# gabrielcheda/optimized-rag

Measured on AMD Instinct MI355X. Metric: queries/sec + p50 retrieve+rerank latency, 1536-d top-k=20, higher is better.
Workload: dtype f16 MFMA + block-scaled bf8 MFMA corrections (fp32 acc) in the cross-encoder; f16 MFMA pass + f64 rescore in the dense leg; f64 BM25 / RRF; 1 GPU; 1000000 docs x 1536-d + BM25 postings (2M-term Zipf vocabulary) + 224-token passage store; batch=256 queries: dense top-100 + BM25 top-100 + RRF -> top-100 -> ms-marco-MiniLM-L-6 cross-encoder (L=256, 25,600 pairs, seeded weights) -> top-20 (BASELINE.json configs[3]); corpus_rows=1000000, rows_per_gpu=1000000, batch_queries=256, pool=100, k=20, parallelism=one rag_retrieve_rerank_dev call per batch, exchange=single process

## Files before the change

optimized-rag_amd/csrc/api.hip:

```cpp
#include "common.h"

#include <cctype>
#include <cmath>
#include <cstdlib>
#include <cstring>

static thread_local std::string g_null_err = "null handle";

static const struct { const char* name; int rag_options::*field; } g_options[] = {
    {"force_level", &rag_options::force_level},         {"stage_growth", &rag_options::stage_growth},
    {"no_smallq", &rag_options::no_smallq},             {"no_second_pass", &rag_options::no_second_pass},
    {"dense_linear_order", &rag_options::dense_linear_order}, {"dense_persist", &rag_options::dense_persist},
    {"bm25_first_ranges", &rag_options::bm25_first_ranges}, {"bm25_no_staging", &rag_options::bm25_no_staging},
    {"bm25_packed", &rag_options::bm25_packed},         {"bm25_plan_slots", &rag_options::bm25_plan_slots},       {"bm25_ws_mb", &rag_options::bm25_ws_mb},
    {"bm25_tail_fold", &rag_options::bm25_tail_fold},     {"bm25_keep_tf", &rag_options::bm25_keep_tf},
    {"sparse_tail_fold", &rag_options::sparse_tail_fold}, {"tokvec_compact_rows", &rag_options::tokvec_compact_rows},
    {"bm25_linear_grid", &rag_options::bm25_linear_grid},            {"bm25_sort_merge", &rag_options::bm25_sort_merge},
    {"no_fork", &rag_options::no_fork},                 {"fork_max_q", &rag_options::fork_max_q},
    {"ce_chunk_tokens", &rag_options::ce_chunk_tokens}, {"ce_mx", &rag_options::ce_mx},
    {"ce_attn_stream", &rag_options::ce_attn_stream},
};
static void options_from_env(rag_options* o) {
    for (const auto& e : g_options) {
        std::string env = "RAG_";
        for (const char* c = e.name; *c; ++c) env += (char)toupper(*c);
        if (const char* v = getenv(env.c_str())) o->*(e.field) = atoi(v);
    }
}
#define DEV_ENTRY(h)                                                                           \
    do {                                                                                      \
        HIP_TRY(h, hipSetDevice((h)->device));                                                \
        (h)->dev_pending = true;                                                              \
    } while (0)
#define HOST_ENTRY(h)                                                                          \
    do {                                                                                      \
        HIP_TRY(h, hipSetDevice((h)->device));                                                \
        if (int rc_ = host_after_dev(h)) return rc_;                                          \
    } while (0)

struct entry_tenants { int tenant; query_tenants qt; };
static int entry_tenants_of(rag_ctx* h, int tenant, const int32_t* tenants_host, int Q, hipStream_t st, entry_tenants* out) {
    *out = {tenant, {nullptr, nullptr}};
    if (tenants_host == nullptr) return RAG_OK;
    const int32_t t0 = std::max(tenants_host[0], -1);
    bool uniform = true;
    for (int q = 1; q < Q && uniform; ++q) uniform = std::max(tenants_host[q], -1) == t0;
    out->tenant = t0;
    return uniform ? RAG_OK : stage_query_tenants(h, tenants_host, Q, st, &out->qt);
}

template <class T>
static int pairwise_cosine_host_t(rag_handle_t h, const T* a, int m, const T* b, int n, int dim, double* out) {
    if (!h) return RAG_ERR_ARG;
    LOCK(h);
    ARG_CHECK(h, m >= 0 && n >= 0 && dim > 0, "bad sizes");
    if (m == 0 || n == 0) return RAG_OK;
    ARG_CHECK(h, a && b && out, "null pointer");
    HOST_ENTRY(h);
    const bool same = (a == b && m == n);
    hipStream_t st = h->stream;
    int rc = stage_reserve(h, stage_size((size_t)m * dim, sizeof(T)) + stage_size(same ? 0 : (size_t)n * dim, sizeof(T)) + stage_size((size_t)m * n, 8));
    if (rc) return rc;
    char* p = h->stage;
    T* ad = stage_take<T>(p, (size_t)m * dim);
    T* bd = same ? ad : stage_take<T>(p, (size_t)n * dim);
    double* od = stage_take<double>(p, (size_t)m * n);
    HIP_TRY(h, hipMemcpyAsync(ad, a, (size_t)m * dim * sizeof(T), hipMemcpyHostToDevice, st));
    if (!same) HIP_TRY(h, hipMemcpyAsync(bd, b, (size_t)n * dim * sizeof(T), hipMemcpyHostToDevice, st));
    if constexpr (sizeof(T) == 8) rc = pairwise_cosine_f64(h, ad, m, bd, n, dim, od, st);
    else rc = pairwise_cosine(h, ad, m, bd, n, dim, od, st);
    if (rc) return rc;
    HIP_TRY(h, hipMemcpyAsync(out, od, (size_t)m * n * sizeof(double), hipMemcpyDeviceToHost, st));
    HIP_TRY(h, hipStreamSynchronize(st));
// ... 1411 lines not shown
```

optimized-rag_amd/csrc/ce_mx.h:

```cpp
#pragma once
#include "common.h"

typedef int mx_v8i __attribute__((ext_vector_type(8)));
typedef int mx_v4i __attribute__((ext_vector_type(4)));

#define MX_TM 384
#define MX_TN 128
#define MX_A_PLANE (MX_TM * 16)
#define MX_B_PLANE (MX_TN * 16)
#define MX_A_STAGE (6 * MX_A_PLANE)
#define MX_B_STAGE (6 * MX_B_PLANE)
#define MX_STAGE (MX_A_STAGE + MX_B_STAGE)
#define MX_STAGES 3
#define MX_LDS (MX_STAGES * MX_STAGE)
#ifndef MX_HI8_TRUNCATE
#define MX_LO_SCALE 2048.0f
#else
#define MX_LO_SCALE (2048.0f * 1.0928961748633879f)
#endif
#define MX_SCALE_A 116
#define MX_SCALE_B 127

__host__ __device__ __forceinline__ int mx_hi_off(int rows, int r, int e) {
    const int j = e >> 4, h = (e >> 2) & 1, i = ((e >> 3) & 1) * 4 + (e & 3);
// ... 29 lines not shown

__device__ __forceinline__ mx_v4i mx_hi8(half8 f0, half8 f1) {
    const mx_v4i a = __builtin_bit_cast(mx_v4i, f0), b = __builtin_bit_cast(mx_v4i, f1);
    return (mx_v4i){mx_top4(a[0], a[1]), mx_top4(b[0], b[1]), mx_top4(a[2], a[3]), mx_top4(b[2], b[3])};
}
__device__ __forceinline__ mx_v8i mx_cat(mx_v4i lo, mx_v4i hi) { return (mx_v8i){lo[0], lo[1], lo[2], lo[3], hi[0], hi[1], hi[2], hi[3]}; }

template <bool SWAP>
__device__ __forceinline__ void mx_block(f32x16& acc, half8 wh0, half8 wh1, mx_v8i w8, half8 xh0, half8 xh1, mx_v8i x8) {
    if (!SWAP) {
        acc = __builtin_amdgcn_mfma_f32_32x32x16_f16(wh0, xh0, acc, 0, 0, 0);
        acc = __builtin_amdgcn_mfma_f32_32x32x16_f16(wh1, xh1, acc, 0, 0, 0);
        acc = __builtin_amdgcn_mfma_scale_f32_32x32x64_f8f6f4(w8, x8, acc, 1, 1, 0, MX_SCALE_A, 0, MX_SCALE_B);
    } else {
        acc = __builtin_amdgcn_mfma_f32_32x32x16_f16(xh0, wh0, acc, 0, 0, 0);
        acc = __builtin_amdgcn_mfma_f32_32x32x16_f16(xh1, wh1, acc, 0, 0, 0);
        acc = __builtin_amdgcn_mfma_scale_f32_32x32x64_f8f6f4(x8, w8, acc, 1, 1, 0, MX_SCALE_B, 0, MX_SCALE_A);
    }
}

__device__ __forceinline__ void mx_bdma(__amdgpu_buffer_rsrc_t rs, unsigned voff, unsigned soff, char* lds_uniform) {
    __builtin_amdgcn_raw_ptr_buffer_load_lds(rs, (__attribute__((address_space(3))) void*)lds_uniform, 16, voff, soff, 0, 0);
}

#define MX_BAR __builtin_amdgcn_s_barrier(); __builtin_amdgcn_sched_barrier(0);
#ifndef MX_ISSUE_W
#define MX_ISSUE_W(...) mx_bdma(__VA_ARGS__)
#endif
#ifndef MX_ISSUE_X
#define MX_ISSUE_X(...) mx_bdma(__VA_ARGS__)
#endif
#ifndef MX_BLOCK
#define MX_BLOCK(SWAP, ...) mx_block<SWAP>(__VA_ARGS__)
#endif
#ifndef MX_W_HI8
#define MX_W_HI8(h0, h1, lo) mx_hi8(h0, h1)
#endif
#ifndef MX_READ_A_IF
#define MX_READ_A_IF(b) true
#endif
#ifndef MX_STEP_WAIT
#define MX_STEP_WAIT "s_waitcnt vmcnt(6)"
#endif

struct mx_tile_iter {
    int n_ft, n_tt, xcd, n_slots, work;
    __device__ __forceinline__ int tt() const { return (work / n_ft) * 8 + xcd; }
    __device__ __forceinline__ int ft() const { return work % n_ft; }
    __device__ __forceinline__ bool valid() const { return tt() < n_tt; }
};

struct mx_stream {
    __amdgpu_buffer_rsrc_t w_rs, x_cur, x_nxt;
    unsigned w_cur, w_nxt, voff;
    int wid, ring, nk, a_off, b_off;
    bool has_next;
    char* smem;
};

#define MX_PIECE(S, k, st_, ws_, xrs_, ks_)                                                                               \
    {                                                                                                                     \
        const int p_ = (S).wid + 8 * (k);                                                                                 \
        if (p_ < 36) { MX_ISSUE_W((S).w_rs, (S).voff, (ws_) + (ks_) * MX_A_STAGE + p_ * 1024, (st_) + p_ * 1024); }         \
        else { MX_ISSUE_X(xrs_, (S).voff, (ks_) * MX_B_STAGE + (p_ - 36) * 1024, (st_) + p_ * 1024); }                     \
    }

template <bool SWAP>
__device__ __forceinline__ void mx_ksteps(f32x16 (&acc)[6], const mx_stream& S, bool first) {
    const int nk = S.nk;
    for (int t = 0; t < nk; ++t) {
        if (first || t > 0) asm volatile(MX_STEP_WAIT ::: "memory");
        MX_BAR
        const char* st = S.smem + ((S.ring + t) % MX_STAGES) * MX_STAGE;
        const int u2 = t + 2;
        const bool nx_ = u2 >= nk && S.has_next;
        const unsigned ks_ = (unsigned)(u2 < nk ? u2 : (S.has_next ? u2 - nk : nk - 1));
        char* const dst = S.smem + ((S.ring + u2) % MX_STAGES) * MX_STAGE;
        const unsigned wsrc = nx_ ? S.w_nxt : S.w_cur;
        const __amdgpu_buffer_rsrc_t xsrc = nx_ ? S.x_nxt : S.x_cur;
        const half8 xh0 = *reinterpret_cast<const half8*>(st + S.b_off);
        const half8 xh1 = *reinterpret_cast<const half8*>(st + S.b_off + 2 * MX_B_PLANE);
        const mx_v4i xl = *reinterpret_cast<const mx_v4i*>(st + S.b_off + 4 * MX_B_PLANE);
        half8 wh0[2], wh1[2];
        mx_v4i wl[2];
#define MX_READ_A(b, s)                                                                                               \
        wh0[s] = *reinterpret_cast<const half8*>(st + S.a_off + (b) * 512);                                            \
        wh1[s] = *reinterpret_cast<const half8*>(st + S.a_off + (b) * 512 + 2 * MX_A_PLANE);                           \
        wl[s] = *reinterpret_cast<const mx_v4i*>(st + S.a_off + (b) * 512 + 4 * MX_A_PLANE);
        MX_READ_A(0, 0)
        MX_READ_A(1, 1)
        const mx_v8i x8 = SWAP ? mx_cat(xl, mx_hi8(xh0, xh1)) : mx_cat(mx_hi8(xh0, xh1), xl);
#pragma unroll
        for (int b = 0; b < 6; ++b) {
            const mx_v4i w8h = MX_W_HI8(wh0[b & 1], wh1[b & 1], wl[b & 1]);
            const mx_v8i w8 = SWAP ? mx_cat(w8h, wl[b & 1]) : mx_cat(wl[b & 1], w8h);
            __builtin_amdgcn_sched_barrier(0);
            __builtin_amdgcn_s_setprio(1);
            MX_BLOCK(SWAP, acc[b], wh0[b & 1], wh1[b & 1], w8, xh0, xh1, x8);
            __builtin_amdgcn_s_setprio(0);
            __builtin_amdgcn_sched_barrier(0);
            if (b + 2 < 6 && MX_READ_A_IF(b + 2)) { MX_READ_A(b + 2, b & 1) }
            MX_PIECE(S, b, dst, wsrc, xsrc, ks_)
        }
#undef MX_READ_A
    }
}

template <class EPI>
__device__ __forceinline__ void mx_gemm_loop(const char* __restrict__ W, const char* __restrict__ X, int nk, int n_ft,
                                             int n_tt, char* smem, EPI& epi) {
    const int tid = threadIdx.x, lane = tid & 63;
    const int wid = __builtin_amdgcn_readfirstlane(tid >> 6);
    const int wm = wid >> 2, wn = wid & 3;
    mx_tile_iter it{n_ft, n_tt, (int)(blockIdx.x & 7), (int)(gridDim.x >> 3), (int)(blockIdx.x >> 3)};
    if (!it.valid()) return;
    const unsigned a_tile_b = (unsigned)nk * MX_A_STAGE, b_tile_b = (unsigned)nk * MX_B_STAGE;
    mx_stream S;
    S.voff = (unsigned)lane * 16u;
    S.wid = wid;
    S.nk = nk;
    S.smem = smem;
    S.ring = 0;
    S.w_rs = __builtin_amdgcn_make_buffer_rsrc(const_cast<char*>(W), 0, (int)((size_t)n_ft * a_tile_b), 0x00020000);
    S.x_cur = __builtin_amdgcn_make_buffer_rsrc(const_cast<char*>(X + (size_t)it.tt() * b_tile_b), 0, (int)b_tile_b, 0x00020000);
    S.x_nxt = S.x_cur;
    S.w_cur = (unsigned)it.ft() * a_tile_b;
    S.w_nxt = S.w_cur;
    S.has_next = false;
    S.a_off = (lane >> 5) * MX_A_PLANE + (wm * 192 + (lane & 31)) * 16;
    S.b_off = MX_A_STAGE + (lane >> 5) * MX_B_PLANE + (wn * 32 + (lane & 31)) * 16;
#pragma unroll
    for (int u = 0; u < 2; ++u) {
        char* st_ = smem + u * MX_STAGE;
#pragma unroll
        for (int k = 0; k < 6; ++k) MX_PIECE(S, k, st_, S.w_cur, S.x_cur, (unsigned)u)
    }
    epi.prepare(smem + MX_LDS);
    asm volatile("s_waitcnt lgkmcnt(0)" ::: "memory");
    MX_BAR
    for (bool first = true;; first = false) {
        {
            mx_tile_iter nx = it;
            nx.work += it.n_slots;
            S.has_next = nx.valid();
            if (S.has_next) {
                S.w_nxt = (unsigned)nx.ft() * a_tile_b;
                S.x_nxt = __builtin_amdgcn_make_buffer_rsrc(const_cast<char*>(X + (size_t)nx.tt() * b_tile_b), 0, (int)b_tile_b, 0x00020000);
            }
        }
        const bool swap = epi.swap_for(it.ft());
        f32x16 acc[6];
#pragma unroll
        for (int b = 0; b < 6; ++b)
#pragma unroll
            for (int r = 0; r < 16; ++r) acc[b][r] = 0.f;
        if (swap) mx_ksteps<true>(acc, S, first);
        else mx_ksteps<false>(acc, S, first);
        asm volatile("s_waitcnt vmcnt(0)" ::: "memory");
        MX_BAR
        epi(acc, it.tt(), it.ft(), swap, smem + MX_LDS);
        if (!S.has_next) break;
        it.work += it.n_slots;
        S.w_cur = S.w_nxt;
        S.x_cur = S.x_nxt;
        S.ring = (S.ring + nk) % MX_STAGES;
    }
    asm volatile("s_waitcnt vmcnt(0)" ::: "memory");
}

#define MX_PARAM_OFF 2048
__device__ __forceinline__ void mx_stage_params(float* dst, const float* __restrict__ src, int n) {
    for (int i = threadIdx.x; i < n; i += blockDim.x) dst[i] = src[i];
}
typedef unsigned mx_u2 __attribute__((ext_vector_type(2)));
typedef unsigned mx_u4 __attribute__((ext_vector_type(4)));

__device__ __forceinline__ size_t mx_img_base(int64_t m, int k, int nk) { return ((size_t)(m >> 7) * nk + (k >> 5)) * MX_B_STAGE; }

typedef short mx_s2 __attribute__((ext_vector_type(2)));
typedef float mx_f2 __attribute__((ext_vector_type(2)));
#ifndef MX_HI8_TRUNCATE
__device__ __forceinline__ void mx_split4(float v0, float v1, float v2, float v3, mx_u2& hi, unsigned& lo) {
    const half4 h = {(half_t)v0, (half_t)v1, (half_t)v2, (half_t)v3};
    hi = __builtin_bit_cast(mx_u2, h);
    float neg1;
    asm volatile("s_mov_b32 %0, 0xbf800000" : "=s"(neg1));
    const float l0 = __builtin_fmaf((float)h[0], neg1, v0), l1 = __builtin_fmaf((float)h[1], neg1, v1);
    const float l2 = __builtin_fmaf((float)h[2], neg1, v2), l3 = __builtin_fmaf((float)h[3], neg1, v3);
// ... 307 lines not shown
                const half8 rj = (q >> 1) ? r1 : r0;
                const half4 rh = (q & 1) ? (half4){rj[4], rj[5], rj[6], rj[7]} : (half4){rj[0], rj[1], rj[2], rj[3]};
                const unsigned rl = rl4[(q & 1) * 2 + (q >> 1)];
                float res[4];
                mx_join4(rh, rl, res);
                acc[b][q * 4] += bv.x + res[0];
                acc[b][q * 4 + 1] += bv.y + res[1];
                acc[b][q * 4 + 2] += bv.z + res[2];
                acc[b][q * 4 + 3] += bv.w + res[3];
                sm += (acc[b][q * 4] + acc[b][q * 4 + 1]) + (acc[b][q * 4 + 2] + acc[b][q * 4 + 3]);
            }
        }
        const float m_l = sm * (1.0f / 96.0f);
#pragma unroll
        for (int b = 0; b < 6; ++b)
#pragma unroll
            for (int r = 0; r < 16; ++r) { const float d = acc[b][r] - m_l; sq = fmaf(d, d, sq); }
        const float m_o = __shfl_xor(m_l, 32), sq_o = __shfl_xor(sq, 32);
        const float m_w = 0.5f * (m_l + m_o);
        const float sq_w = (sq + sq_o) + (m_l - m_o) * (m_l - m_o) * 48.0f;
        if (hh == 0) { st_sum[li] = m_w; st_sq[li] = sq_w; }
        asm volatile("s_waitcnt lgkmcnt(0)" ::: "memory");
        MX_BAR
        const float m_p = pr_sum[li], sq_p = pr_sq[li];
        const float mu = 0.5f * (m_w + m_p);
        const float var = ((sq_w + sq_p) + (m_w - m_p) * (m_w - m_p) * 96.0f) * (1.0f / H);
        const float rs = 1.0f / sqrtf(var + eps);
#pragma unroll
        for (int b = 0; b < 6; ++b) {
            const int f0 = wm * 192 + b * 32;
            float v[16];
#pragma unroll
            for (int q = 0; q < 4; ++q) {
                const float4 gv = *reinterpret_cast<const float4*>(gamma + f0 + 8 * q + 4 * hh);
                const float4 be = *reinterpret_cast<const float4*>(beta + f0 + 8 * q + 4 * hh);
                v[q * 4] = fmaf(acc[b][q * 4] - mu, rs * gv.x, be.x);
                v[q * 4 + 1] = fmaf(acc[b][q * 4 + 1] - mu, rs * gv.y, be.y);
                v[q * 4 + 2] = fmaf(acc[b][q * 4 + 2] - mu, rs * gv.z, be.z);
                v[q * 4 + 3] = fmaf(acc[b][q * 4 + 3] - mu, rs * gv.w, be.w);
            }
            mx_store_block(tile + (size_t)(f0 >> 5) * MX_B_STAGE, trow, hh, v);
        }
    }
};

template <class EPI>
__global__ __launch_bounds__(512) void mx_gemm_kernel(const char* __restrict__ W, const char* __restrict__ X, int nk, int n_ft,
                                                       const int32_t* __restrict__ m_packed, EPI epi) {
    extern __shared__ __attribute__((aligned(16))) char smem[];
    const int n_tt = (m_packed[0] + MX_TN - 1) / MX_TN;
    mx_gemm_loop(W, X, nk, n_ft, n_tt, smem, epi);
}
#define MX_KERNEL_LDS (MX_LDS + MX_PARAM_OFF + 6144)
```

optimized-rag_amd/csrc/common.h:

```cpp
#pragma once
#include <hip/hip_runtime.h>
#include <stdint.h>
#include <mutex>
#include <string>
#include <unordered_map>
#include <vector>

#include "../../include/rag_hip.h"

typedef _Float16 half_t;
typedef _Float16 half8 __attribute__((ext_vector_type(8)));
typedef _Float16 half4 __attribute__((ext_vector_type(4)));
typedef float f32x4 __attribute__((ext_vector_type(4)));
typedef float f32x16 __attribute__((ext_vector_type(16)));

#define RAG_CAND_CAP 4096
#define RAG_STAGE0_ROWS 2048
#define RAG_STAGE_GROWTH 8
#define RAG_TILE 256
#define RAG_BK 64
#define RAG_MAX_K 256
#define RAG_SCALE_LOG2 7

#define RAG_PROF_STAGES 3
struct rag_ce_model;
struct rag_bm25_index;
struct rag_ctx;

template <class T>
struct dev_buf {
    dev_buf() = default;
    dev_buf(dev_buf&& o) noexcept : p_(o.p_), n_(o.n_) { o.p_ = nullptr; o.n_ = 0; }
    dev_buf& operator=(dev_buf&& o) noexcept {
        if (this != &o) { reset(); p_ = o.p_; n_ = o.n_; o.p_ = nullptr; o.n_ = 0; }
        return *this;
    }
    ~dev_buf() { reset(); }
    void reset() {
        if (p_) (void)hipFree(p_);
        p_ = nullptr;
        n_ = 0;
    }
    int alloc(rag_ctx* h, size_t n);
    int reserve(rag_ctx* h, size_t n) { return n <= n_ ? RAG_OK : alloc(h, n); }
    operator T*() const { return p_; }
    T* get() const { return p_; }
    size_t size() const { return n_; }

private:
    T* p_ = nullptr;
    size_t n_ = 0;
};

struct rag_options {
    int force_level = 0;
    int stage_growth = 0;
    int no_smallq = 0;
    int no_second_pass = 0;
    int dense_persist = 0;
    int dense_linear_order = 0;
    int bm25_first_ranges = 0;
    int bm25_no_staging = 0;
    int bm25_linear_grid = 0;
    int bm25_sort_merge = 0;
    int bm25_plan_slots = 0;
    int bm25_ws_mb = 0;
    int bm25_packed = 0;
    int bm25_keep_tf = 0;
    int bm25_tail_fold = 0;
    int sparse_tail_fold = 0;
    int tokvec_compact_rows = 0;
    int no_fork = 0;
    int fork_max_q = 0;
    int ce_chunk_tokens = 0;
    int ce_mx = 0;
    int ce_attn_stream = 0;
};

struct dense_ws {
    dev_buf<half_t> q16;
    dev_buf<uint64_t> cand;
    dev_buf<unsigned> cnt;
    dev_buf<float> tau;
    dev_buf<float> bound;
    dev_buf<int> n_sorted;
    int alloc(rag_ctx* h, size_t rows, hipStream_t st);
};

struct rag_index_mem {
    dev_buf<float> emb32;
    dev_buf<half_t> emb16;
    dev_buf<int64_t> ids;
    dev_buf<int32_t> tenants;
    dev_buf<int> bad_rows;
    dev_buf<char> scan_scores;
    dev_buf<int32_t> tenant_tiles;
    dev_buf<int32_t> vis;
};
struct rag_device_mem : rag_index_mem {
    dev_buf<double> side_scores;
    dev_buf<double> temporal;
    dev_buf<char> lin_ws;
    dense_ws ws;
    dev_buf<float> q32;
    dev_buf<double> exact;
    dev_buf<int> flag;
    dev_buf<int> scan_list;
    dev_buf<int> stats;
    dense_ws ws_ovf;
    dev_buf<int> ovf_list;
    dev_buf<char> stage;
    dev_buf<uint16_t> tok;
    dev_buf<uint8_t> tok_hi;
    dev_buf<int32_t> tok_len;
    dev_buf<int> tok_bad;
    dev_buf<char> pipe_ws;
    dev_buf<int32_t> qten;
    dev_buf<int32_t> union_tiles;
    dev_buf<half_t> tv;
    dev_buf<uint8_t> tv8;
    dev_buf<int64_t> tv_off;
    dev_buf<int> tv_bad;
    dev_buf<char> tv_ws;
};

struct rag_ctx : rag_device_mem {
    int device = 0;
    int n_cu = 0;
    int dim = 0;
    int dim_pad = 0;
    hipStream_t stream = nullptr;
    hipStream_t side_stream = nullptr;
    hipEvent_t ev_fork = nullptr, ev_join = nullptr;
    std::string err;
    rag_options opt;
    bool profiling = false;
    void* comm = nullptr;
    int comm_rank = 0, comm_world = 1;

    int64_t n_rows = 0, id_base = 0;
    bool index_loaded = false;
    int64_t n_reserved = 0;
    double temporal_absmax = 0.0;
    struct { bool on = false; int Q = 0; int64_t n_rows = 0; int tenant = -1; std::vector<int32_t> tenants; } lin_begun;
    std::unordered_map<int32_t, std::pair<int64_t, int>> tenant_span;
    std::unordered_map<int32_t, std::vector<int32_t>> tenant_lists;
    int64_t tenant_rows = 0;
    int64_t n_deleted = 0;
    bool bm25_stale = false;
    bool bm25_compacted = false;

    bool dev_pending = false;
    int ws_q = 0;
    int q16_dirty = 0;
    std::mutex mu;

    struct prof_spans { std::vector<std::pair<hipEvent_t, hipEvent_t>> ev; int used = 0; };
    prof_spans prof[RAG_PROF_STAGES];
    rag_dense_stats last_stats = {};
    bool last_stats_valid = false;
    int last_q = 0, last_k = 0, last_stages = 0, last_shortlist = 0;
    double last_eps = 0;

    rag_bm25_index* bm25 = nullptr;
    rag_bm25_index* sparse = nullptr;
    bool sparse_stale = false;
    bool sparse_compacted = false;
    int64_t tok_rows = 0;
    int tok_L = 0;
    int64_t tv_docs = 0, tv_rows = 0;
    int64_t tv_docs_cap = 0, tv_rows_cap = 0;
    int tv_dim = 0;
    int tv_form = 0;
    bool tv_stale = false;
    int pair_format = RAG_PAIR_BERT;
    int attr_dense_emit_lds[2][2][2] = {}, attr_dense_persist_lds[2] = {}, attr_dense_select_lds = 0, attr_bm25_lds = 0;
    int attr_ce_gemm_lds = 0, attr_ce_mx_lds = 0;
    int attr_ce_attn_lds[2][3] = {};
    int attr_ce_attn64_lds = 0;
    int attr_ce_attn64s_lds = 0;
    int attr_m3_gemm_lds = 0;
    int attr_m3_compact_lds = 0;
    rag_ce_model* ce = nullptr;
    rag_ce_model* emb = nullptr;
};

#define HIP_TRY(h, expr)                                                                      \
    do {                                                                                      \
        hipError_t _e = (expr);                                                               \
        if (_e != hipSuccess) {                                                               \
            (h)->err = std::string(#expr) + ": " + hipGetErrorString(_e);                     \
            return RAG_ERR_HIP;                                                               \
        }                                                                                     \
    } while (0)

template <class T>
int dev_buf<T>::alloc(rag_ctx* h, size_t n) {
    reset();
    HIP_TRY(h, hipMalloc(&p_, n * sizeof(T)));
    n_ = n;
    return RAG_OK;
}

inline int dense_ws::alloc(rag_ctx* h, size_t rows, hipStream_t st) {
    int rc;
    if ((rc = q16.alloc(h, rows * h->dim_pad))) return rc;
    if ((rc = cand.alloc(h, rows * RAG_CAND_CAP))) return rc;
    if ((rc = cnt.alloc(h, rows))) return rc;
    if ((rc = tau.alloc(h, 2 * rows))) return rc;
    if ((rc = bound.alloc(h, rows))) return rc;
    if ((rc = n_sorted.alloc(h, rows))) return rc;
    HIP_TRY(h, hipMemsetAsync(q16, 0, rows * h->dim_pad * sizeof(half_t), st));
    return RAG_OK;
}

#define LOCK(h) std::lock_guard<std::mutex> lock_((h)->mu)

enum { PLANE_EMB32, PLANE_EMB16, PLANE_IDS, PLANE_TENANTS, PLANE_TEMPORAL, PLANE_VIS, PLANE_TOK, PLANE_TOK_HI, PLANE_TOK_LEN };
template <class F>
static int for_each_row_plane(const rag_ctx* h, F&& f) {
    int rc;
    if ((rc = f(PLANE_EMB32, &rag_device_mem::emb32, (int64_t)h->dim))) return rc;
    if ((rc = f(PLANE_EMB16, &rag_device_mem::emb16, (int64_t)h->dim_pad))) return rc;
    if ((rc = f(PLANE_IDS, &rag_device_mem::ids, (int64_t)1))) return rc;
    if ((rc = f(PLANE_TENANTS, &rag_device_mem::tenants, (int64_t)1))) return rc;
    if ((rc = f(PLANE_TEMPORAL, &rag_device_mem::temporal, (int64_t)1))) return rc;
    if ((rc = f(PLANE_VIS, &rag_device_mem::vis, (int64_t)1))) return rc;
    if ((rc = f(PLANE_TOK, &rag_device_mem::tok, (int64_t)h->tok_L))) return rc;
    if ((rc = f(PLANE_TOK_HI, &rag_device_mem::tok_hi, (int64_t)h->tok_L))) return rc;
    return f(PLANE_TOK_LEN, &rag_device_mem::tok_len, (int64_t)1);
// ... 328 lines not shown
```

optimized-rag_amd/csrc/cross_encoder.hip:

```cpp
#include "common.h"
#include "ce_mx.h"
#include <type_traits>

#include <cmath>
#include <cstdlib>
#include <cstring>

struct ce_chunk_bufs {
    dev_buf<int32_t> ids, tt, lens;
    dev_buf<int32_t> clen;
    dev_buf<int32_t> pair_off, row_off, row_pair, row_att, m_packed;
    dev_buf<int32_t> sid, stt;
    dev_buf<float> logits;
};

struct ce_ws_base {
    int pairs = 0, L = 0;
    int64_t tokens = 0;
    ce_chunk_bufs io;
    bool fits(int P, int L_) const { return P <= pairs && L_ == L; }
};
struct ce_split_ws : ce_ws_base {
    dev_buf<float> y32;
    dev_buf<half_t> x16, q16, kf16, vf16, ctx16, h16;
};
struct ce_mx_ws : ce_ws_base {
    dev_buf<char> x8, ctx8, h8;
    dev_buf<char> xc8, cc8, hc8;
    dev_buf<int32_t> m_cls;
    dev_buf<half_t> qf16, kf16, vf16;
};

struct ce_heads {
    int tok_dim = 0, tok_pad = 0;
    dev_buf<half_t> tok_w;
    dev_buf<float> tok_b;
    dev_buf<float> lex_w;
    float lex_b = 0.f;
    dev_buf<half_t> x16;
    dev_buf<float> raw;
    int64_t x16_tokens = 0, raw_tokens = 0;
};
struct ce_multi {
    float* lex;
    float* tok;
    int64_t* row_off;
    int64_t tok_cap;
};

struct rag_ce_model {
    rag_ce_config cfg;
    ce_heads heads;
    bool embed = false;
    int normalize = 1;
    int pool_cls = 0;
    int d_head = 32;
    int out_width = 1;
    dev_buf<float> word, pos, type, emb_ln_g, emb_ln_b;
    struct Layer {
        dev_buf<half_t> wqkv, wo, w1, w2;
        dev_buf<char> wqkv8, wo8, w18, w28;
        dev_buf<float> bqkv, bo, b1, b2;
        dev_buf<float> ln1_g, ln1_b, ln2_g, ln2_b;
    };
    std::vector<Layer> layers;
    dev_buf<float> wp, bp, wc, bc;
    dev_buf<float> wpT;
    bool mx_ok = false;
    bool mx_default = true;
    ce_split_ws split;
    ce_mx_ws mx;
};

#define CE_BM 128
#define CE_BN 256
#define CE_BK 32
#define CE_W_TILE (CE_BM * 128)
#define CE_X_TILE (CE_BN * 128)
#define CE_STAGE_BYTES (CE_W_TILE + CE_X_TILE)
#define SPLIT_IDX(c) ((((c) >> 5) << 6) + ((c) & 31))
#define CE_GEMM_LDS (3 * CE_STAGE_BYTES)
// ... 1255 lines not shown
        launch(m3_lexical_kernel, dim3((unsigned)(((int64_t)c.P * c.L_in + 3) / 4)), dim3(256), 0, st, x16, io.pair_off, io.clen, c.P, c.L_in, H,
               hd.lex_w, hd.lex_b, c.lex);
    if (c.tok) {
        if (int rc = raise_lds(h, h->attr_m3_gemm_lds, CE_GEMM_LDS, ce_gemm_kernel<EPI_F32>)) return rc;
        launch(ce_gemm_kernel<EPI_F32>, dim3(ce_gemm_grid(h)), dim3(512), CE_GEMM_LDS, st, hd.tok_w, x16, hd.tok_pad, H, hd.tok_b, nullptr, hd.raw,
               nullptr, nullptr, nullptr, (size_t)0, H, m->cfg.heads, io.m_packed, (int)w.tokens);
        launch(m3_tok_scatter_kernel, dim3((unsigned)(((int64_t)c.P * c.L + 3) / 4)), dim3(256), 0, st, hd.raw, hd.tok_pad, hd.tok_dim, io.m_packed,
               io.row_pair, io.pair_off, io.clen, c.row_off, c.tok_cap, c.tok);
    }
    return RAG_OK;
}

static int ce_forward_chunk(rag_ctx* h, rag_ce_model* m, const ce_chunk& c, hipStream_t st) {
    ce_split_ws& w = m->split;
    const ce_chunk_bufs& io = w.io;
    const int H = m->cfg.hidden, F = m->cfg.ffn, P = c.P, L = c.L;
    const int64_t M = (int64_t)P * L;
    int rc;
    if ((rc = raise_lds(h, h->attr_ce_gemm_lds, CE_GEMM_LDS, ce_gemm_kernel<EPI_QKV>, ce_gemm_kernel<EPI_GELU>, ce_gemm_kernel<EPI_RESID>,
                        ce_gemm_kernel<EPI_QKV64>)))
        return rc;
    chunk_prologue(w, c, 16, st);
    rc = per_lane_dispatch(h, H, [&](auto per) {
        launch(ce_embed_ln_kernel<decltype(per)::value>, dim3((unsigned)((M + 3) / 4)), dim3(256), 0, st, io.ids, io.tt, m->word, m->pos,
               m->type, m->emb_ln_g, m->emb_ln_b, io.m_packed, io.row_pair, io.pair_off, L, H, m->cfg.vocab_size, m->cfg.max_pos, (float)m->cfg.ln_eps, w.x16);
    });
    if (rc) return rc;
    for (const auto& ly : m->layers) {
        if (m->d_head == 64) {
            ce_gemm<EPI_QKV64>(h, m, st, ly.wqkv, w.x16, 3 * H, H, ly.bqkv, nullptr, nullptr, w.q16, w.kf16, w.vf16, kv_plane_halfs(w.tokens, H));
            rc = launch_attention64(h, m, w, c, st);
        } else {
            ce_gemm<EPI_QKV>(h, m, st, ly.wqkv, w.x16, 3 * H, H, ly.bqkv, nullptr, nullptr, w.q16, w.kf16, w.vf16, kv_plane_halfs(w.tokens, H));
            rc = L == 32 ? launch_attention<1, false>(h, m, w, w.q16, w.kf16, w.vf16, w.ctx16, c, st)
                         : launch_attention<2, false>(h, m, w, w.q16, w.kf16, w.vf16, w.ctx16, c, st);
        }
        if (rc) return rc;
        ce_gemm<EPI_RESID>(h, m, st, ly.wo, w.ctx16, H, H, ly.bo, w.x16, w.y32, nullptr);
        if ((rc = ce_layernorm(h, m, ly.ln1_g, ly.ln1_b, M, st))) return rc;
        ce_gemm<EPI_GELU>(h, m, st, ly.w1, w.x16, F, H, ly.b1, nullptr, nullptr, w.h16);
        ce_gemm<EPI_RESID>(h, m, st, ly.w2, w.h16, H, F, ly.b2, w.x16, w.y32, nullptr);
        if ((rc = ce_layernorm(h, m, ly.ln2_g, ly.ln2_b, M, st))) return rc;
    }
    if (m->embed) {
        if (c.out) launch(ce_meanpool_kernel<false>, dim3(P), dim3(256), 0, st, w.x16, io.pair_off, io.clen, L, H, m->normalize, m->pool_cls, c.out);
        if (c.lex || c.tok)
            if ((rc = heads_chunk(h, m, w, w.x16, c, st))) return rc;
    } else
        launch(ce_pool_classify_kernel<false>, dim3(P), dim3(256), 0, st, w.x16, m->wp, m->bp, m->wc, m->bc, io.pair_off, H, c.out);
    HIP_TRY(h, hipGetLastError());
    return RAG_OK;
}

static int mx_ensure_ws(rag_ctx* h, rag_ce_model* m, int P, int L, hipStream_t st) {
    ce_mx_ws& w = m->mx;
    if (w.fits(P, L)) return RAG_OK;
    int rc;
    if ((rc = ws_renew(h, w, P, L, m->out_width, st))) return rc;
    const size_t H = m->cfg.hidden, F = m->cfg.ffn, rows = (size_t)w.tokens, kv = kv_plane_halfs(w.tokens, H);
    const size_t cls_rows = (size_t)round_up((int64_t)P, MX_TN);
    if ((rc = alloc_zeroed(h, w.x8, rows * H * 3, st))) return rc;
    if ((rc = alloc_zeroed(h, w.ctx8, rows * H * 3, st))) return rc;
    if ((rc = alloc_zeroed(h, w.h8, rows * F * 3, st))) return rc;
    if ((rc = alloc_zeroed(h, w.xc8, cls_rows * H * 3, st))) return rc;
    if ((rc = alloc_zeroed(h, w.cc8, cls_rows * H * 3, st))) return rc;
    if ((rc = alloc_zeroed(h, w.hc8, cls_rows * F * 3, st))) return rc;
    if ((rc = w.m_cls.alloc(h, 1))) return rc;
    if ((rc = alloc_zeroed(h, w.qf16, 2 * kv, st))) return rc;
    if ((rc = alloc_zeroed(h, w.kf16, 2 * kv, st))) return rc;
    if ((rc = alloc_zeroed(h, w.vf16, 2 * kv, st))) return rc;
    w.pairs = P;
    w.L = L;
    return RAG_OK;
}

template <class EPI>
static void mx_gemm(rag_ctx* h, hipStream_t st, const char* W, const char* X, int nk, int n_ft, const int32_t* rows, EPI epi) {
    launch(mx_gemm_kernel<EPI>, dim3(ce_gemm_grid(h)), dim3(512), MX_KERNEL_LDS, st, W, X, nk, n_ft, rows, epi);
}

static void mx_qkv(rag_ctx* h, const rag_ce_model* m, const rag_ce_model::Layer& ly, hipStream_t st, int ft_base, int n_ft, const char* X,
                   const int32_t* rows, const int32_t* row_map = nullptr, int n_map = 0) {
    const ce_mx_ws& w = m->mx;
    const int nk = m->cfg.hidden / 32;
    mx_gemm(h, st, ly.wqkv8 + (size_t)ft_base * nk * MX_A_STAGE, X, nk, n_ft, rows,
            mx_epi_qkv{w.qf16, w.kf16, w.vf16, kv_plane_halfs(w.tokens, m->cfg.hidden), ly.bqkv, (int)(w.tokens >> 4), ft_base, w.io.row_att,
                       row_map, n_map});
}

static void mx_layer_tail(rag_ctx* h, const rag_ce_model* m, const rag_ce_model::Layer& ly, hipStream_t st, const char* attn, char* x,
                          char* ffn, const int32_t* rows) {
    const int H = m->cfg.hidden, F = m->cfg.ffn;
    const float eps = (float)m->cfg.ln_eps;
    mx_gemm(h, st, ly.wo8, attn, H / 32, 1, rows, mx_epi_ln{x, ly.bo, ly.ln1_g, ly.ln1_b, eps});
    mx_gemm(h, st, ly.w18, x, H / 32, F / MX_TM, rows, mx_epi_gelu{ffn, ly.b1, F / 32});
    mx_gemm(h, st, ly.w28, ffn, F / 32, 1, rows, mx_epi_ln{x, ly.b2, ly.ln2_g, ly.ln2_b, eps});
}

static int mx_forward_chunk(rag_ctx* h, rag_ce_model* m, const ce_chunk& c, hipStream_t st) {
    ce_mx_ws& w = m->mx;
    const ce_chunk_bufs& io = w.io;
    const int H = m->cfg.hidden, P = c.P, L = c.L;
    int rc;
    if ((rc = raise_lds(h, h->attr_ce_mx_lds, MX_KERNEL_LDS, mx_gemm_kernel<mx_epi_qkv>, mx_gemm_kernel<mx_epi_gelu>, mx_gemm_kernel<mx_epi_ln>)))
        return rc;
    chunk_prologue(w, c, m->embed ? 16 : 4, st);
    launch(mx_embed_ln_kernel, dim3((unsigned)(((int64_t)P * L + MX_EMB_ROWS - 1) / MX_EMB_ROWS)), dim3(256), 0, st, io.ids, io.tt, m->word,
           m->pos, m->type, m->emb_ln_g, m->emb_ln_b, io.m_packed, io.row_pair, io.row_off, L, m->cfg.vocab_size, (float)m->cfg.ln_eps, w.x8);
    half_t* const ctx = reinterpret_cast<half_t*>(w.ctx8.get());
    const dim3 gather_grid((unsigned)(((int64_t)P * 72 + 255) / 256));
    bool cls_tail = false;
    for (int l = 0; l < m->cfg.layers; ++l) {
        const auto& ly = m->layers[l];
        cls_tail = !m->embed && l == m->cfg.layers - 1;
        if (cls_tail) {
            launch(mx_gather_rows_kernel, gather_grid, dim3(256), 0, st, w.x8, nullptr, io.row_off, P, H / 32, w.xc8, nullptr, w.m_cls);
            mx_qkv(h, m, ly, st, 1, 2, w.x8, io.m_packed);
            mx_qkv(h, m, ly, st, 0, 1, w.xc8, w.m_cls, io.pair_off, P);
        } else
            mx_qkv(h, m, ly, st, 0, 3, w.x8, io.m_packed);
        const int qblocks = cls_tail ? 1 : 1 << 20;
        rc = L <= 256 ? launch_attention<1, true>(h, m, w, w.qf16, w.kf16, w.vf16, ctx, c, st, qblocks)
                      : launch_attention<2, true>(h, m, w, w.qf16, w.kf16, w.vf16, ctx, c, st, qblocks);
        if (rc) return rc;
        if (cls_tail) {
            launch(mx_gather_rows_kernel, gather_grid, dim3(256), 0, st, w.ctx8, nullptr, io.row_off, P, H / 32, w.cc8, nullptr, w.m_cls);
            mx_layer_tail(h, m, ly, st, w.cc8, w.xc8, w.hc8, w.m_cls);
        } else
            mx_layer_tail(h, m, ly, st, w.ctx8, w.x8, w.h8, io.m_packed);
    }
    const char* const cls = cls_tail ? w.xc8 : w.x8;
    if (m->embed) {
        if (c.out)
            launch(ce_meanpool_kernel<true>, dim3(P), dim3(256), 0, st, reinterpret_cast<const half_t*>(w.x8.get()), io.pair_off, io.clen, L, H,
                   m->normalize, m->pool_cls, c.out);
        if (c.lex || c.tok) {
            launch(m3_mx_to_split_kernel, dim3((unsigned)(((int64_t)P * L * H + 255) / 256)), dim3(256), 0, st, w.x8, io.m_packed, H, m->heads.x16);
            if ((rc = heads_chunk(h, m, w, m->heads.x16, c, st))) return rc;
        }
    } else if (cls_tail && P >= 512)
        launch(mx_pool_classify_kernel, dim3((unsigned)((P + POOL_PB - 1) / POOL_PB)), dim3(256), 0, st, cls, m->wpT, m->bp, m->wc, m->bc, P, H, c.out);
    else
        launch(ce_pool_classify_kernel<true>, dim3(P), dim3(256), 0, st, reinterpret_cast<const half_t*>(cls), m->wp, m->bp, m->wc, m->bc,
               cls_tail ? nullptr : io.row_off.get(), H, c.out);
    HIP_TRY(h, hipGetLastError());
    return RAG_OK;
}

static bool ce_use_mx(const rag_ctx* h, const rag_ce_model* m) {
    return m->mx_ok && (h->opt.ce_mx > 0 || (h->opt.ce_mx == 0 && m->mx_default));
}

static int heads_ensure_ws(rag_ctx* h, rag_ce_model* m, int64_t tokens, bool use_mx, bool tok, hipStream_t st) {
    ce_heads& hd = m->heads;
    const size_t H = m->cfg.hidden;
    int rc;
    if (use_mx && hd.x16_tokens != tokens) {
        HIP_TRY(h, hipStreamSynchronize(st));
// ... 207 lines not shown
```

Before: 1064 queries/sec.

## Fuse cross-encoder FFN up and down GEMMs into one persistent kernel

```diff
diff --git a/optimized-rag_amd/csrc/api.hip b/optimized-rag_amd/csrc/api.hip
--- a/optimized-rag_amd/csrc/api.hip
+++ b/optimized-rag_amd/csrc/api.hip
@@ -18,7 +18,7 @@
     {"bm25_linear_grid", &rag_options::bm25_linear_grid},            {"bm25_sort_merge", &rag_options::bm25_sort_merge},
     {"no_fork", &rag_options::no_fork},                 {"fork_max_q", &rag_options::fork_max_q},
     {"ce_chunk_tokens", &rag_options::ce_chunk_tokens}, {"ce_mx", &rag_options::ce_mx},
-    {"ce_attn_stream", &rag_options::ce_attn_stream},
+    {"ce_attn_stream", &rag_options::ce_attn_stream},   {"ce_ffn_fused", &rag_options::ce_ffn_fused},
 };
 static void options_from_env(rag_options* o) {
     for (const auto& e : g_options) {
diff --git a/optimized-rag_amd/csrc/ce_mx.h b/optimized-rag_amd/csrc/ce_mx.h
--- a/optimized-rag_amd/csrc/ce_mx.h
+++ b/optimized-rag_amd/csrc/ce_mx.h
@@ -105,20 +105,21 @@
 
 struct mx_stream {
     __amdgpu_buffer_rsrc_t w_rs, x_cur, x_nxt;
+    __amdgpu_buffer_rsrc_t w_rs_nxt;
     unsigned w_cur, w_nxt, voff;
     int wid, ring, nk, a_off, b_off;
     bool has_next;
     char* smem;
 };
 
-#define MX_PIECE(S, k, st_, ws_, xrs_, ks_)                                                                               \
+#define MX_PIECE(S, k, st_, wrs_, ws_, xrs_, ks_)                                                                         \
     {                                                                                                                     \
         const int p_ = (S).wid + 8 * (k);                                                                                 \
-        if (p_ < 36) { MX_ISSUE_W((S).w_rs, (S).voff, (ws_) + (ks_) * MX_A_STAGE + p_ * 1024, (st_) + p_ * 1024); }         \
+        if (p_ < 36) { MX_ISSUE_W(wrs_, (S).voff, (ws_) + (ks_) * MX_A_STAGE + p_ * 1024, (st_) + p_ * 1024); }            \
         else { MX_ISSUE_X(xrs_, (S).voff, (ks_) * MX_B_STAGE + (p_ - 36) * 1024, (st_) + p_ * 1024); }                     \
     }
 
-template <bool SWAP>
+template <bool SWAP, bool WSWITCH = false>
 __device__ __forceinline__ void mx_ksteps(f32x16 (&acc)[6], const mx_stream& S, bool first) {
     const int nk = S.nk;
     for (int t = 0; t < nk; ++t) {
@@ -130,6 +131,7 @@
         const unsigned ks_ = (unsigned)(u2 < nk ? u2 : (S.has_next ? u2 - nk : nk - 1));
         char* const dst = S.smem + ((S.ring + u2) % MX_STAGES) * MX_STAGE;
         const unsigned wsrc = nx_ ? S.w_nxt : S.w_cur;
+        const __amdgpu_buffer_rsrc_t wrs = WSWITCH && nx_ ? S.w_rs_nxt : S.w_rs;
         const __amdgpu_buffer_rsrc_t xsrc = nx_ ? S.x_nxt : S.x_cur;
         const half8 xh0 = *reinterpret_cast<const half8*>(st + S.b_off);
         const half8 xh1 = *reinterpret_cast<const half8*>(st + S.b_off + 2 * MX_B_PLANE);
@@ -153,7 +155,7 @@
             __builtin_amdgcn_s_setprio(0);
             __builtin_amdgcn_sched_barrier(0);
             if (b + 2 < 6 && MX_READ_A_IF(b + 2)) { MX_READ_A(b + 2, b & 1) }
-            MX_PIECE(S, b, dst, wsrc, xsrc, ks_)
+            MX_PIECE(S, b, dst, wrs, wsrc, xsrc, ks_)
         }
 #undef MX_READ_A
     }
@@ -186,7 +188,7 @@
     for (int u = 0; u < 2; ++u) {
         char* st_ = smem + u * MX_STAGE;
 #pragma unroll
-        for (int k = 0; k < 6; ++k) MX_PIECE(S, k, st_, S.w_cur, S.x_cur, (unsigned)u)
+        for (int k = 0; k < 6; ++k) MX_PIECE(S, k, st_, S.w_rs, S.w_cur, S.x_cur, (unsigned)u)
     }
     epi.prepare(smem + MX_LDS);
     asm volatile("s_waitcnt lgkmcnt(0)" ::: "memory");
@@ -600,3 +602,109 @@
     mx_gemm_loop(W, X, nk, n_ft, n_tt, smem, epi);
 }
 #define MX_KERNEL_LDS (MX_LDS + MX_PARAM_OFF + 6144)
+
+#define MX_FFN_GELU_OFF (3 * 384 * 4)
+#define MX_FFN_LDS (MX_LDS + MX_PARAM_OFF + MX_FFN_GELU_OFF + 6144)
+__host__ __device__ __forceinline__ size_t mx_ffn_slot_bytes(int ffn) { return (size_t)MX_TN * ffn * 3; }
+
+__device__ __forceinline__ void mx_ffn_loop(const char* W1, const char* W2, int n_up, int n_tt, char* smem, mx_epi_gelu gelu,
+                                            const mx_epi_ln& ln) {
+    const int tid = threadIdx.x, lane = tid & 63;
+    const int wid = __builtin_amdgcn_readfirstlane(tid >> 6);
+    const int wm = wid >> 2, wn = wid & 3;
+    const int xcd = (int)(blockIdx.x & 7), n_slots = (int)(gridDim.x >> 3);
+    int work = (int)(blockIdx.x >> 3);
+    if (work * 8 + xcd >= n_tt) return;
+    constexpr int NK_UP = 384 / 32;
+    const int nk_dn = n_up * (MX_TM / 32);
+    const unsigned up_tile_b = NK_UP * MX_A_STAGE, x_tile_b = NK_UP * MX_B_STAGE, slot_b = (unsigned)mx_ffn_slot_bytes(nk_dn * 32);
+    const char* const X = ln.x8;
+    gelu.h8 += (size_t)blockIdx.x * slot_b;
+    const __amdgpu_buffer_rsrc_t w1_rs = __builtin_amdgcn_make_buffer_rsrc(const_cast<char*>(W1), 0, (int)((size_t)n_up * up_tile_b), 0x00020000);
+    const __amdgpu_buffer_rsrc_t w2_rs = __builtin_amdgcn_make_buffer_rsrc(const_cast<char*>(W2), 0, (int)((size_t)nk_dn * MX_A_STAGE), 0x00020000);
+    const __amdgpu_buffer_rsrc_t slot_rs = __builtin_amdgcn_make_buffer_rsrc(gelu.h8, 0, (int)slot_b, 0x00020000);
+    mx_stream S;
+    S.voff = (unsigned)lane * 16u;
+    S.wid = wid;
+    S.nk = NK_UP;
+    S.smem = smem;
+    S.ring = 0;
+    S.w_rs = S.w_rs_nxt = w1_rs;
+    S.x_cur = __builtin_amdgcn_make_buffer_rsrc(const_cast<char*>(X + (size_t)(work * 8 + xcd) * x_tile_b), 0, (int)x_tile_b, 0x00020000);
+    S.x_nxt = S.x_cur;
+    S.w_cur = S.w_nxt = 0;
+    S.has_next = false;
+    S.a_off = (lane >> 5) * MX_A_PLANE + (wm * 192 + (lane & 31)) * 16;
+    S.b_off = MX_A_STAGE + (lane >> 5) * MX_B_PLANE + (wn * 32 + (lane & 31)) * 16;
+#pragma unroll
+    for (int u = 0; u < 2; ++u) {
+        char* st_ = smem + u * MX_STAGE;
+#pragma unroll
+        for (int k = 0; k < 6; ++k) MX_PIECE(S, k, st_, S.w_rs, S.w_cur, S.x_cur, (unsigned)u)
+    }
+    ln.prepare(smem + MX_LDS);
+    gelu.prepare(smem + MX_LDS + MX_FFN_GELU_OFF);
+    asm volatile("s_waitcnt lgkmcnt(0)" ::: "memory");
+    MX_BAR
+    int item = 0;
+    for (bool first = true;;) {
+        const bool down = item == n_up;
+        const int tt = work * 8 + xcd;
+        if (!down) {
+            const bool to_down = item + 1 == n_up;
+            S.has_next = !(to_down && n_up == 1);
+            S.w_rs_nxt = to_down ? w2_rs : w1_rs;
+            S.w_nxt = to_down ? 0u : (unsigned)(item + 1) * up_tile_b;
+            S.x_nxt = to_down ? slot_rs : S.x_cur;
+        } else {
+            const int tt_n = (work + n_slots) * 8 + xcd;
+            S.has_next = tt_n < n_tt;
+            if (S.has_next) {
+                S.w_rs_nxt = w1_rs;
+                S.w_nxt = 0;
+                S.x_nxt = __builtin_amdgcn_make_buffer_rsrc(const_cast<char*>(X + (size_t)tt_n * x_tile_b), 0, (int)x_tile_b, 0x00020000);
+            }
+        }
+        f32x16 acc[6];
+#pragma unroll
+        for (int b = 0; b < 6; ++b)
+#pragma unroll
+            for (int r = 0; r < 16; ++r) acc[b][r] = 0.f;
+        mx_ksteps<false, true>(acc, S, first);
+        asm volatile("s_waitcnt vmcnt(0)" ::: "memory");
+        MX_BAR
+        if (down) {
+            ln(acc, tt, 0, false, smem + MX_LDS);
+            if (!S.has_next) break;
+            work += n_slots;
+            item = 0;
+        } else {
+            gelu(acc, 0, item, false, smem + MX_LDS + MX_FFN_GELU_OFF);
+            ++item;
+        }
+        S.ring = (S.ring + S.nk) % MX_STAGES;
+        S.nk = item == n_up ? nk_dn : NK_UP;
+        S.w_rs = S.w_rs_nxt;
+        S.w_cur = S.w_nxt;
+        S.x_cur = S.x_nxt;
+        first = !S.has_next;
+        if (first) {
+            asm volatile("s_waitcnt vmcnt(0)" ::: "memory");
+            MX_BAR
+#pragma unroll
+            for (int u = 0; u < 2; ++u) {
+                char* st_ = smem + ((S.ring + u) % MX_STAGES) * MX_STAGE;
+#pragma unroll
+                for (int k = 0; k < 6; ++k) MX_PIECE(S, k, st_, S.w_rs, S.w_cur, S.x_cur, (unsigned)u)
+            }
+        }
+    }
+    asm volatile("s_waitcnt vmcnt(0)" ::: "memory");
+}
+
+__global__ __launch_bounds__(512) void mx_ffn_kernel(const char* __restrict__ W1, const char* __restrict__ W2, int n_up,
+                                                      const int32_t* __restrict__ m_packed, mx_epi_gelu gelu, mx_epi_ln ln) {
+    extern __shared__ __attribute__((aligned(16))) char smem[];
+    const int n_tt = (m_packed[0] + MX_TN - 1) / MX_TN;
+    mx_ffn_loop(W1, W2, n_up, n_tt, smem, gelu, ln);
+}
diff --git a/optimized-rag_amd/csrc/common.h b/optimized-rag_amd/csrc/common.h
--- a/optimized-rag_amd/csrc/common.h
+++ b/optimized-rag_amd/csrc/common.h
@@ -74,6 +74,7 @@
     int fork_max_q = 0;
     int ce_chunk_tokens = 0;
     int ce_mx = 0;
+    int ce_ffn_fused = 0;
     int ce_attn_stream = 0;
 };
 
@@ -175,7 +176,7 @@
     bool tv_stale = false;
     int pair_format = RAG_PAIR_BERT;
     int attr_dense_emit_lds[2][2][2] = {}, attr_dense_persist_lds[2] = {}, attr_dense_select_lds = 0, attr_bm25_lds = 0;
-    int attr_ce_gemm_lds = 0, attr_ce_mx_lds = 0;
+    int attr_ce_gemm_lds = 0, attr_ce_mx_lds = 0, attr_ce_ffn_lds = 0;
     int attr_ce_attn_lds[2][3] = {};
     int attr_ce_attn64_lds = 0;
     int attr_ce_attn64s_lds = 0;
diff --git a/optimized-rag_amd/csrc/cross_encoder.hip b/optimized-rag_amd/csrc/cross_encoder.hip
--- a/optimized-rag_amd/csrc/cross_encoder.hip
+++ b/optimized-rag_amd/csrc/cross_encoder.hip
@@ -27,6 +27,7 @@
 struct ce_mx_ws : ce_ws_base {
     dev_buf<char> x8, ctx8, h8;
     dev_buf<char> xc8, cc8, hc8;
+    dev_buf<char> ffn_slots;
     dev_buf<int32_t> m_cls;
     dev_buf<half_t> qf16, kf16, vf16;
 };
@@ -1388,26 +1389,40 @@
     return RAG_OK;
 }
 
+#define MX_FFN_SLOT_CAP ((size_t)192 << 20)
+static size_t mx_ffn_slots_bytes(const rag_ctx* h, const rag_ce_model* m) { return (size_t)ce_gemm_grid(h) * mx_ffn_slot_bytes(m->cfg.ffn); }
+static bool mx_ffn_fused(const rag_ctx* h, const rag_ce_model* m) {
+    return h->opt.ce_ffn_fused > 0 || (h->opt.ce_ffn_fused == 0 && mx_ffn_slots_bytes(h, m) <= MX_FFN_SLOT_CAP);
+}
+
+static int mx_ensure_ffn(rag_ctx* h, rag_ce_model* m, hipStream_t st) {
+    ce_mx_ws& w = m->mx;
+    int rc;
+    if (mx_ffn_fused(h, m)) return w.ffn_slots ? RAG_OK : alloc_zeroed(h, w.ffn_slots, mx_ffn_slots_bytes(h, m), st);
+    if (w.h8) return RAG_OK;
+    const size_t F = m->cfg.ffn;
+    if ((rc = alloc_zeroed(h, w.h8, (size_t)w.tokens * F * 3, st))) return rc;
+    return alloc_zeroed(h, w.hc8, (size_t)round_up((int64_t)w.pairs, MX_TN) * F * 3, st);
+}
+
 static int mx_ensure_ws(rag_ctx* h, rag_ce_model* m, int P, int L, hipStream_t st) {
     ce_mx_ws& w = m->mx;
-    if (w.fits(P, L)) return RAG_OK;
+    if (w.fits(P, L)) return mx_ensure_ffn(h, m, st);
     int rc;
     if ((rc = ws_renew(h, w, P, L, m->out_width, st))) return rc;
-    const size_t H = m->cfg.hidden, F = m->cfg.ffn, rows = (size_t)w.tokens, kv = kv_plane_halfs(w.tokens, H);
+    const size_t H = m->cfg.hidden, rows = (size_t)w.tokens, kv = kv_plane_halfs(w.tokens, H);
     const size_t cls_rows = (size_t)round_up((int64_t)P, MX_TN);
     if ((rc = alloc_zeroed(h, w.x8, rows * H * 3, st))) return rc;
     if ((rc = alloc_zeroed(h, w.ctx8, rows * H * 3, st))) return rc;
-    if ((rc = alloc_zeroed(h, w.h8, rows * F * 3, st))) return rc;
     if ((rc = alloc_zeroed(h, w.xc8, cls_rows * H * 3, st))) return rc;
     if ((rc = alloc_zeroed(h, w.cc8, cls_rows * H * 3, st))) return rc;
-    if ((rc = alloc_zeroed(h, w.hc8, cls_rows * F * 3, st))) return rc;
     if ((rc = w.m_cls.alloc(h, 1))) return rc;
     if ((rc = alloc_zeroed(h, w.qf16, 2 * kv, st))) return rc;
     if ((rc = alloc_zeroed(h, w.kf16, 2 * kv, st))) return rc;
     if ((rc = alloc_zeroed(h, w.vf16, 2 * kv, st))) return rc;
     w.pairs = P;
     w.L = L;
-    return RAG_OK;
+    return mx_ensure_ffn(h, m, st);
 }
 
 template <class EPI>
@@ -1429,6 +1444,11 @@
     const int H = m->cfg.hidden, F = m->cfg.ffn;
     const float eps = (float)m->cfg.ln_eps;
     mx_gemm(h, st, ly.wo8, attn, H / 32, 1, rows, mx_epi_ln{x, ly.bo, ly.ln1_g, ly.ln1_b, eps});
+    if (mx_ffn_fused(h, m)) {
+        launch(mx_ffn_kernel, dim3(ce_gemm_grid(h)), dim3(512), MX_FFN_LDS, st, ly.w18, ly.w28, F / MX_TM, rows,
+               mx_epi_gelu{m->mx.ffn_slots, ly.b1, F / 32}, mx_epi_ln{x, ly.b2, ly.ln2_g, ly.ln2_b, eps});
+        return;
+    }
     mx_gemm(h, st, ly.w18, x, H / 32, F / MX_TM, rows, mx_epi_gelu{ffn, ly.b1, F / 32});
     mx_gemm(h, st, ly.w28, ffn, F / 32, 1, rows, mx_epi_ln{x, ly.b2, ly.ln2_g, ly.ln2_b, eps});
 }
@@ -1440,6 +1460,7 @@
     int rc;
     if ((rc = raise_lds(h, h->attr_ce_mx_lds, MX_KERNEL_LDS, mx_gemm_kernel<mx_epi_qkv>, mx_gemm_kernel<mx_epi_gelu>, mx_gemm_kernel<mx_epi_ln>)))
         return rc;
+    if ((rc = raise_lds(h, h->attr_ce_ffn_lds, MX_FFN_LDS, mx_ffn_kernel))) return rc;
     chunk_prologue(w, c, m->embed ? 16 : 4, st);
     launch(mx_embed_ln_kernel, dim3((unsigned)(((int64_t)P * L + MX_EMB_ROWS - 1) / MX_EMB_ROWS)), dim3(256), 0, st, io.ids, io.tt, m->word,
            m->pos, m->type, m->emb_ln_g, m->emb_ln_b, io.m_packed, io.row_pair, io.row_off, L, m->cfg.vocab_size, (float)m->cfg.ln_eps, w.x8);
```

Result: faster. 1077 queries/sec (median of 6 runs) (+1.2%).
